# winddori2002/DEX-TTS

Hardware: AMD Instinct MI355X
Metric: mel-frames/s at n_timesteps=50, 80-ch mel (sampler only); RTF (higher is better)
Workload: dtype bf16; 1 GPU; gedex_b1: gedex_lj B=1/GPU T=512 n_timesteps=50 (BASELINE.json configs[1]); global_batch=1, frames=512, hipgraph=True, parallelism=1 GPU

## Files before the change

### dex_tts_amd/csrc/dex_api.hip

```cpp
#include <hip/hip_runtime.h>
#include <cstdlib>

#include <cmath>
#include <cstdarg>
#include <atomic>
#include <cstdio>
#include <mutex>
#include <cstring>
#include <map>
#include <unordered_map>
#include <string_view>
#include <string>
#include <vector>

#include "../../include/dex_amd.h"
#include "kernels.h"
#include "weight_store.h"

using namespace dex;

namespace dex {
namespace {
const char* const KNOB_NAMES[] = {
    "DEX_CONV_STREAM", "DEX_CONV_PP", "DEX_CONV_SKIP_DEAD", "DEX_H_BF16", "DEX_ATTN_SEPARATE", "DEX_ATTN_Q64", "DEX_ATTN_Q64_TAIL", "DEX_ATTN_Q64_HALF", "DEX_DIT_XCDS", "DEX_ATTN_GENERIC", "DEX_RES2", "DEX_LP_INTER", "DEX_DIT_CHAIN",
    "DEX_DIT_CLUSTER", "DEX_DIT_CLUSTER_LOCAL", "DEX_ATTN_X_LP", "DEX_RES_X_LP", "DEX_CAT_LP", "DEX_XCD_MAP", "DEX_DEBUG_DROP_HANDOFF", "DEX_PATCH_FUSED",
    "DEX_CONV_DOWN", "DEX_CONVT_UP", "DEX_DEBUG_PLAN",
    "DEX_ATTN_SHARED_W8", "DEX_CONVT_MT", "DEX_CONVT_WGS", "DEX_CONV_DOWN_WGS", "DEX_CONV_REGW", "DEX_CONV_REGW_RES", "DEX_CONV_SMALL_MAX", "DEX_CONV_TH8",
    "DEX_CONV_W8", "DEX_DWCONV_CAP", "DEX_FINAL_CAP", "DEX_FIRST_CAP", "DEX_FIRST_MFMA", "DEX_GEMM_NWALK", "DEX_NWALK_SPLIT", "DEX_NWALK_BM", "DEX_POS_COL", "DEX_POS_COL_MIN",
    "DEX_POS_CT", "DEX_REGW_MIN_TILES", "DEX_REGW_WGS", "DEX_ROWCHAIN64", "DEX_ROWCHAIN64A", "DEX_TIV_CAP", "DEX_TV_CHAIN", "DEX_TIV_FOLD", "DEX_LINATTN_NSUB", "DEX_TV_FOLD", "DEX_OUT2_MIN", "DEX_NWALK_DMA"};
constexpr int N_KNOBS = (int)(sizeof(KNOB_NAMES) / sizeof(KNOB_NAMES[0]));
int knob_parse(const char* e) {
    if (!e) return KNOB_UNSET;
    char* end = nullptr;
    const long v = strtol(e, &end, 10);
    if (end == e) {
        static bool warned = false;
        if (!warned) { warned = true; fprintf(stderr, "libdexamd: ignoring a DEX_* knob whose value '%s' is not an integer\n", e); }
        return KNOB_UNSET;
    }
    return (int)v;
}
struct KnobSnapshot {
    int v[N_KNOBS];
    KnobSnapshot() { for (int i = 0; i < N_KNOBS; ++i) v[i] = knob_parse(getenv(KNOB_NAMES[i])); }
};
thread_local const KnobSnapshot* t_knobs = nullptr;
struct WsplitScope {
    bool prev;
    explicit WsplitScope(bool on) : prev(g_lp_wsplit) { g_lp_wsplit = on; }
    ~WsplitScope() { g_lp_wsplit = prev; }
};
struct KnobScope {
    const KnobSnapshot* prev;
    explicit KnobScope(const KnobSnapshot* k) : prev(t_knobs) { t_knobs = k; }
    ~KnobScope() { t_knobs = prev; }
};
}
static int knob_index(const char* name) {
    static const std::unordered_map<std::string_view, int> idx = [] {
        std::unordered_map<std::string_view, int> m;
        for (int i = 0; i < N_KNOBS; ++i) m.emplace(KNOB_NAMES[i], i);
        return m;
    }();
    const auto it = idx.find(std::string_view(name));
    return it == idx.end() ? -1 : it->second;
}
int knob(const char* name) {
    if (t_knobs) {
        const int i = knob_index(name);
        if (i >= 0) return t_knobs->v[i];
    }
    return knob_parse(getenv(name));
}
}
static_assert(PREC_FP32 == DEX_PREC_FP32 && PREC_BF16 == DEX_PREC_BF16 && PREC_FP16 == DEX_PREC_FP16 && PREC_FP16X2 == DEX_PREC_FP16X2, "kernels.h mirrors DexPrecision");

namespace {
void xcd_map_probe();

struct TD { float* p; int ld; int coff; int C; int lp = 0; };

struct ResW { const float *w1, *b1, *g1, *be1, *w2, *b2, *g2, *be2, *wr, *br, *mlp_w, *mlp_b; int cin, cout; };
// ... 856 lines not shown
        if (tail) {
            tail->H2 = s.h2; tail->gn_stats = st2; tail->gamma = w.g2; tail->beta = w.be2;
            tail->res = resptr; tail->ldres = ldres; tail->resb = resb; tail->res_under_mask = under ? 1 : 0;
            tail->res_lp = (head && head->xout_lp && resptr == X.p) ? 1 : 0;
            tail->mask = mask; tail->mask_ws = s.mask_ws; tail->mask_bstride = P.d.T; tail->W = s.W; tail->Xout = out;
            tail->h2_bf16 = h2b ? 1 : 0;
            return;
        }
        gn_apply(s.h2, w.cout, npix, s.W, s.mask_ws, st2, w.g2, w.be2, nullptr, resptr, ldres, resb, under, out);
    }

    bool lp_inter_cur = false;
    bool cat_lp = false;
    IGemmP final_gemm(int mask_ws, float* out, int ldo, int ocoff) {
        const DexConfig& c = x->cfg;
        const int hid = c.dit_hidden, mid = mid_dim(c);
        const bool fuse_lnf = x->lp() && ln_fusable(hid);
        const int s2c = c.dit_stride * c.dit_stride * mid;
        IGemmP fl = base_gemm(fuse_lnf ? P.tok : P.xn, hid, 0, P.Hf, P.Wt, hid, x->fl_w, s2c, x->fl_b, out, ldo, ocoff);
        if (fuse_lnf) { fl.ln_shift = P.fin_mod; fl.ln_scale = P.fin_mod + hid; fl.ln_step_stride = 2L * hid; }
        { auto it = x->frag_of().find(x->fl_w); fl.Wfrag = (it != x->frag_of().end()) ? it->second : nullptr; }
        fl.unpatch_s = c.dit_stride; fl.unpatch_C = mid; fl.OHf = P.Hm; fl.OWf = P.Wm;
        fl.c_bstride = (long)P.Hm * P.Wm * ldo;
        fl.outmask = mask; fl.outmask_ws = mask_ws;
        return fl;
    }
    bool linattn_fused(int C) const { return x->lp() && (C == 64 || C == 128) && linattn_fused_supported(C); }
    void linattn(const LinW& w, const StageBuf& s, const TD& X, float* out, int ldo, int ocoff, const LinKvCtxP* tail = nullptr, bool out_lp = false,
                 void* out2_lp = nullptr, int ldo2 = 0, int ocoff2 = 0) {
        const long npix = s.npix; const int B = P.d.B;
        if (linattn_fused(X.C)) {
            int nsub = 1;
            while (nsub < 4 && (npix + 128 * nsub - 1) / (128 * nsub) * B > 192) nsub *= 2;
            {
                const int ncu = device_cus();
                const long slots = (long)(X.C == 64 ? 2 : 1) * ncu;
                if ((npix + 127) / 128 * B >= 2 * slots) {
                    long best = -1;
                    for (int n = 1; n <= 8; ++n) {
                        const long wgs = (npix + 128L * n - 1) / (128L * n) * B;
                        const long cost = (wgs + slots - 1) / slots * n;
                        if (best < 0 || cost <= best) { best = cost; nsub = n; }
                    }
                }
                const int forced = knob_or("DEX_LINATTN_NSUB", 0);
                if (forced > 0) nsub = forced;
            }
            const int nblk = (int)((npix + 128L * nsub - 1) / (128L * nsub));
            LinKvCtxP k{};
            if (tail) k = *tail;
            k.X = X.p; k.ldx = X.ld; k.x_coff = X.coff; k.xb = npix * X.ld; k.npix = (int)npix; k.C = X.C; k.Wkv = w.wkv_lp[x->lpi()];
            k.wkv_lo_off = x->lpi() == 2 ? 384L * X.C : 0;
            k.nsub = nsub; k.nblk = nblk; k.part_m = s.pm; k.part_s = s.ps; k.part_c = s.pc; k.B = B;
            const bool xlp = k.H2 && k.Xout && lp_inter_cur && linattn_out2_lp_out_supported((int)npix, B) && !knob_off("DEX_ATTN_X_LP");
            k.xout_lp = xlp ? 1 : 0;
            run("linattn_kvctx", 2.0 * npix * B * (256.0 * X.C + 128 * 32), (tail ? (tail->h2_bf16 ? 10.0 : 12.0) - (xlp ? 2.0 : 0.0) : 4.0) * npix * X.C * B, [&] { launch_linattn_kvctx(k, x->precision, st); });
            LinMergeP mg{s.pm, s.ps, s.pc, nblk, w.wout_raw, w.g, X.C, s.mbf, B};
            run("linattn_merge", 2.0 * 128 * 32 * X.C * B, 4.0 * nblk * 4 * 1088 * B, [&] { launch_linattn_merge(mg, x->precision, st); });
            LinOut2P o{X.p, X.ld, X.coff, npix * X.ld, (int)npix, X.C, w.wq_frag[x->lpi()], s.mbf, w.bias_eff, out, ldo, ocoff, npix * ldo, B, out_lp ? 1 : 0,
                       out2_lp, ldo2, ocoff2, npix * ldo2, xlp ? 1 : 0};
            o.wq_lo_off = x->lpi() == 2 ? 128L * X.C : 0;
            run("linattn_out", 4.0 * npix * B * 128.0 * X.C, ((out_lp ? 6.0 : 8.0) - (xlp ? 2.0 : 0.0) + (out2_lp ? 2.0 : 0.0)) * npix * X.C * B, [&] { launch_linattn_out2(o, x->precision, st); });
            return;
        }
        IGemmP g = base_gemm(X.p, X.ld, X.coff, s.H, s.W, X.C, w.wqkv, 384, nullptr, s.qkv, 384, 0);
        gemm("linattn_qkv", g);
        LinAttnCtxP cp{s.qkv, 384, npix * 384, (int)npix, 4, LA_CHUNK, s.nchunks, s.pm, s.ps, s.pc, B};
        run("linattn_ctx", 2.0 * npix * 128 * 32 * B, 4.0 * npix * 384 * B, [&] { launch_linattn_ctx(cp, st); });
        LinAttnCombineP cb{s.pm, s.ps, s.pc, s.nchunks, 4, w.wout_raw, w.g, w.C, s.weff, B};
        run("linattn_combine", 2.0 * 128 * 32 * w.C * B, 4.0 * s.nchunks * 4 * 1100 * B, [&] { launch_linattn_combine(cb, st); });
        IGemmP o = base_gemm(s.qkv, 384, 0, s.H, s.W, 128, s.weff, w.C, w.bias_eff, out, ldo, ocoff);
        o.w_bstride = 128L * w.C;
        o.res = X.p; o.ldres = X.ld; o.res_coff = X.coff; o.res_bstride = npix * X.ld;
        gemm("linattn_out", o);
    }

    void dit(const TD& X, bool mask_input, int mask_ws, float* out, int ldo, int ocoff, const float* in_aff = nullptr) {
        const DexConfig& c = x->cfg;
        const int B = P.d.B, hid = c.dit_hidden, mid = mid_dim(c), N = P.N, mh = mlp_hidden(c);
        DwConvP dw{};
        dw.X = X.p + X.coff; dw.ldx = X.ld; dw.xb = (long)P.Hm * P.Wm * X.ld; dw.Hi = P.Hm; dw.Wi = P.Wm; dw.C = mid;
        dw.k = c.dit_patch; dw.s = c.dit_stride; dw.pad = c.dit_patch / 2; dw.Wd = x->pe_dw; dw.bd = x->pe_db;
        dw.mask = mask_input ? mask : nullptr; dw.mask_ws = mask_ws; dw.mask_bstride = P.d.T;
        dw.Y = P.pe0; dw.Hf = P.Hf; dw.Wt = P.Wt; dw.B = B; dw.aff = in_aff;
        auto pw_lp = x->lp_of().find(x->pe_pw);
        if (patch_fused()) {
            run("patch_embed", 2.0 * B * N * mid * (c.dit_patch * c.dit_patch + hid), 4.0 * B * (P.Hm * P.Wm * mid + N * hid),
                [&] { launch_patch_embed_fused(dw, pw_lp->second, x->pe_pb, P.emb, hid, x->precision, st); });
        } else {
            run("patch_dwconv_silu", 2.0 * B * N * mid * c.dit_patch * c.dit_patch, 4.0 * B * (P.Hm * P.Wm + N) * mid, [&] { launch_dwconv_silu(dw, st); });
            IGemmP pe = base_gemm(P.pe0, mid, 0, P.Hf, P.Wt, mid, x->pe_pw, hid, x->pe_pb, P.emb, hid, 0);
            gemm("patch_pointwise", pe);
        }
        const int G = c.dit_conv_pos_groups, kp = c.dit_conv_pos, cg = hid / G;
        int nsplit = POS_SPLIT, pcg = 0, pcgp = 0;
        if (x->lp() && x->pos_wfrag[x->lpi()]) {
            PosConvP pcd{P.emb, x->pos_wfrag[x->lpi()], P.pos_part, P.Hf, P.Wt, hid, G, B};
            run("pos_conv", 2.0 * B * N * (double)kp * kp * cg * hid, 8.0 * B * N * hid + 2.0 * kp * kp * cg * hid, [&] { launch_pos_conv_direct(pcd, x->precision, st); });
            nsplit = 1;
        } else {
            const int cgp = (cg % 32) ? 64 : cg;
            const float* src = P.emb;
            if (cgp != cg) {
                run("pos_group_pad", 0, 8.0 * B * N * hid, [&] { launch_group_pad(P.emb, P.emb_pad, (long)B * N, G, cg, cgp, st); });
                src = P.emb_pad;
            }
// ... 821 lines not shown
```

### dex_tts_amd/csrc/kernels.h

```cpp
#pragma once
#include <hip/hip_runtime.h>
#include <stdint.h>

namespace dex {

constexpr int KNOB_UNSET = -2147483647 - 1;
int knob(const char* name);
inline int knob_or(const char* name, int dflt) { const int v = knob(name); return v == KNOB_UNSET ? dflt : v; }
inline bool knob_off(const char* name) { return knob(name) == 0; }
inline bool knob_set(const char* name) { return knob(name) != KNOB_UNSET; }
inline int device_cus() {
    static const int n = [] { int dev = 0, v = 0; (void)hipGetDevice(&dev); (void)hipDeviceGetAttribute(&v, hipDeviceAttributeMultiprocessorCount, dev); return v > 0 ? v : 256; }();
    return n;
}

constexpr int GN_SLOTS = 32;
typedef long long gnfix_t;

extern thread_local const char* g_last_symbol;

constexpr int PREC_FP32 = 0, PREC_BF16 = 1, PREC_FP16 = 2, PREC_FP16X2 = 3;
inline bool prec_wsplit(int precision) { return precision == PREC_FP16X2; }
extern thread_local bool g_lp_wsplit;
inline bool prec_is_lp(int precision) { return precision != PREC_FP32; }
// ... 86 lines not shown

struct GnStatsP { const float* X; int ld; long bstride; int npix; int C; int groups; gnfix_t* stats; int B; };
void launch_gn_stats(const GnStatsP& p, hipStream_t st);

struct GnApplyP {
    const float* X; int ldx; long xb;
    float* Y; int ldy; long yb; int y_coff;
    int npix, W, C, groups; const gnfix_t* stats; const float* gamma; const float* beta;
    const float* mask; int mask_ws; long mask_bstride;
    const float* tadd; long tadd_step_stride; int step;
    const float* res; int ldres; long resb; int res_under_mask;
    int B;
};
void launch_gn_apply(const GnApplyP& p, hipStream_t st);

struct FinalP {
    const float* X; long xb; int npix, W, C, groups; const gnfix_t* stats; const float* gamma; const float* beta;
    const float* mask; long mask_bstride;
    const float* wfc; const float* bfc;
    const float* xcur;
    float* denoised;
    float* xnext;
    const float* scal; int scal_stride; int step;
    float* zero_ptr; long zero_n;
    int B;
    int mode; const float* htab; float* dbuf; const float* xhat;
    int x_bf16;
    const int* poison;
};
void launch_final(const FinalP& p, hipStream_t st);
void launch_churn_tables(const float* sigmas, int n, float S_churn, float S_min, float S_max, float S_noise,
                         float* t_hat, float* h, float* ncoef, hipStream_t st);
void launch_add_noise(float* x, const float* noise, const float* ncoef_i, long n, hipStream_t st);
void launch_heun_expand(const float* t_hat, const float* h, int n, float* sig, float* hout, hipStream_t st);

struct LinAttnCtxP { const float* qkv; int ld; long bstride; int n; int heads; int chunk; int nchunks;
                     float* part_m; float* part_s; float* part_c; int B; };
void launch_linattn_ctx(const LinAttnCtxP& p, hipStream_t st);
struct LinAttnCombineP { const float* part_m; const float* part_s; const float* part_c; int nchunks; int heads;
                         const float* Wout;
                         const float* g;
                         int C; float* Weff;
                         int B; };
void launch_linattn_combine(const LinAttnCombineP& p, hipStream_t st);

struct LinKvCtxP { const float* X; int ldx; int x_coff; long xb; int npix; int C; const void* Wkv; int nsub; int nblk;
                   float* part_m; float* part_s; float* part_c; int B;
                   const float* H2; const gnfix_t* gn_stats; const float* gamma; const float* beta;
                   const float* res; int ldres; long resb; int res_under_mask;
                   const float* mask; int mask_ws; long mask_bstride; int W; float* Xout;
                   int h2_bf16;
                   int res_lp;
                   int xout_lp;     long wkv_lo_off = 0;
};
void launch_linattn_kvctx(const LinKvCtxP& p, int precision, hipStream_t st);
struct LinMergeP { const float* part_m; const float* part_s; const float* part_c; int nblk;
                   const float* Wout; const float* g; int C; void* W2; int B; };
void launch_linattn_merge(const LinMergeP& p, int precision, hipStream_t st);
struct LinOut2P { const float* X; int ldx; int x_coff; long xb; int npix; int C; const void* Wq; const void* W2;
                  const float* bias; float* Y; int ldy; int y_coff; long yb; int B;
                  int y_lp;
                  void* Y2; int ldy2; int y2_coff; long y2b;
                  int x_lp;     long wq_lo_off = 0;
                  };
void launch_linattn_out2(const LinOut2P& p, int precision, hipStream_t st);
bool linattn_out2_lp_out_supported(int npix, int B);
bool linattn_fused_supported(int C);

struct DwConvP { const float* X; int ldx; long xb; int Hi, Wi, C; int k, s, pad; const float* Wd; const float* bd;
                 const float* mask; int mask_ws; long mask_bstride;
                 float* Y; int Hf, Wt; int B;
                 const float* aff = nullptr; };
void launch_dwconv_silu(const DwConvP& p, hipStream_t st);
bool patch_embed_fused_supported(int k, int C, int hid, long ntok);
void launch_patch_embed_fused(const DwConvP& p, const void* Wb, const float* bias, float* emb, int hid, int precision, hipStream_t st);

struct PosConvP { const float* X; const void* Wf; float* Y; int Hf, Wt, hid, G, B;
                  int ncol; };
bool pos_conv_direct_supported(int hid, int groups, int kernel, int Hf);
void launch_pos_conv_direct(const PosConvP& p, int precision, hipStream_t st);
struct PosFinishP { const float* part; int nsplit; long split_stride; const float* bias; const float* emb;
                    const float* freq_pos; float* tok; int Hf, Wt, D; int B;
                    int cg, cg_pad; };
void launch_pos_finish(const PosFinishP& p, hipStream_t st);
void launch_group_pad(const float* src, float* dst, long rows, int G, int cg, int cg_pad, hipStream_t st);

struct LnModP { const float* X; float* Y; int rows_per_batch; int D; const float* shift; const float* scale;
                long step_stride; int step; int B; };
void launch_ln_mod(const LnModP& p, hipStream_t st);

struct DitChainP { const float* O; int ksplit; long o_sstride; const float* ml; int heads; int rows_per_batch;
                   float* X; const void *Wp, *W1, *W2, *Wq; const float *bp, *b1, *b2, *bq;
                   const float* ada;
                   const float *next_shift, *next_scale; long next_step_stride;
                   void *Qh, *Kh, *Vt; int Npad; float qscale;
                   const void *Qin, *Kin, *Vin;
                   int qkv_only;
                   int attn_inline;
                   int step; int M; int B; long long* dbg;
                   float* xslab; unsigned* xflag; unsigned epoch; int* xerr;
                   int o_lp;
                   int xcd_map;
                   int xlocal;
                   int xdrop;
                   int tail_row0 = 0, tail_ks = 0;
                   int xcds = 8; };
// ... 154 lines not shown
```

### dex_tts_amd/csrc/linattn_fused.hip

```cpp
#include "kernels.h"
#include "lp_util.h"
#include "kernels_lp.h"

namespace dex {
namespace DEX_LP_NS {

typedef float f32x16 __attribute__((ext_vector_type(16)));
typedef unsigned short u16;
union LFrag { uint4 u; lp8 v; };
constexpr float LOG2E_F = 1.4426950408889634f;


template <int C, bool PRO, int FL = -1>
__global__ __launch_bounds__(256) __attribute__((amdgpu_waves_per_eu(C == 64 ? 2 : 1, C == 64 ? 2 : 8))) void linattn_kvctx_kernel(const LinKvCtxP p) {
    constexpr int LDW = C + 8, KS = C / 16;
    extern __shared__ __attribute__((aligned(16))) u16 smem_la[];
    u16* Ws = smem_la;
    const int tid = threadIdx.x, lane = tid & 63, wave = tid >> 6;
    const int i = lane & 31, hh = lane >> 5;
    const int blk = blockIdx.x, b = blockIdx.y;
    const u16* Wg = reinterpret_cast<const u16*>(p.Wkv);
    {
        uint4 wr[C / 8];
#pragma unroll
        for (int j = 0; j < C / 8; ++j) {
            const int it = tid + 256 * j;
            wr[j] = *reinterpret_cast<const uint4*>(Wg + (long)(it / (C / 8)) * C + (it % (C / 8)) * 8);
        }
#pragma unroll
        for (int j = 0; j < C / 8; ++j) {
            const int it = tid + 256 * j;
            *reinterpret_cast<uint4*>(Ws + (it / (C / 8)) * LDW + (it % (C / 8)) * 8) = wr[j];
        }
#ifdef DEX_LP_WSPLIT
#pragma unroll
        for (int j = 0; j < C / 8; ++j) {
            const int it = tid + 256 * j;
            wr[j] = *reinterpret_cast<const uint4*>(Wg + p.wkv_lo_off + (long)(it / (C / 8)) * C + (it % (C / 8)) * 8);
        }
#pragma unroll
        for (int j = 0; j < C / 8; ++j) {
            const int it = tid + 256 * j;
            *reinterpret_cast<uint4*>(Ws + 256 * LDW + (it / (C / 8)) * LDW + (it % (C / 8)) * 8) = wr[j];
        }
#endif
    }
    const float* X = PRO ? p.H2 + (long)b * p.npix * C : p.X + (long)b * p.xb + p.x_coff;
    const int ldx = PRO ? C : p.ldx;
    const float* R = (PRO && p.res) ? p.res + (long)b * p.resb : nullptr;
    const float* mrow = PRO ? p.mask + (long)b * p.mask_bstride : nullptr;
    const int px_base = (blk * 4 + wave) * p.nsub * 32;

    f32x16 ctxT[4];
    float m_run[4], s_run[4];
#pragma unroll
    for (int h = 0; h < 4; ++h) {
        m_run[h] = -INFINITY; s_run[h] = 0.f;
#pragma unroll
        for (int r = 0; r < 16; ++r) ctxT[h][r] = 0.f;
    }
    float4 xa[KS], xc[KS], ra[PRO ? KS : 1], rc[PRO ? KS : 1];
    float mkv = 1.f;
    float ga_pre = 0.f, be_pre = 0.f;
    if constexpr (PRO) { if (tid < C) { ga_pre = p.gamma[tid]; be_pre = p.beta[tid]; } }
    const bool hb = FL >= 0 ? (FL & 1) != 0 : (PRO && p.h2_bf16 != 0);
    const bool rlp = FL >= 0 ? (FL & 2) != 0 : (PRO && p.res_lp != 0);
    const bool xlp = FL >= 0 ? (FL & 4) != 0 : (p.xout_lp != 0);
    const unsigned short* Rh = (PRO && p.res) ? reinterpret_cast<const unsigned short*>(p.res) + (long)b * p.resb : nullptr;
    const unsigned short* Xh = PRO ? reinterpret_cast<const unsigned short*>(p.H2) + (long)b * p.npix * C : nullptr;
    {
        const int pxr = min(px_base + i, p.npix - 1);
        const float* xr = X + (long)pxr * ldx + hh * 8;
        if (hb) {
#pragma unroll
            for (int ks = 0; ks < KS; ++ks) { xa[ks] = *reinterpret_cast<const float4*>(Xh + (long)pxr * C + hh * 8 + ks * 16); xc[ks] = xa[ks]; }
        } else {
#pragma unroll
            for (int ks = 0; ks < KS; ++ks) {
                xa[ks] = *reinterpret_cast<const float4*>(xr + ks * 16);
                xc[ks] = *reinterpret_cast<const float4*>(xr + ks * 16 + 4);
            }
        }
        if constexpr (PRO) {
            if (R) {
                if (rlp) {
#pragma unroll
                    for (int ks = 0; ks < KS; ++ks) { ra[ks] = *reinterpret_cast<const float4*>(Rh + (long)pxr * p.ldres + hh * 8 + ks * 16); rc[ks] = ra[ks]; }
                } else {
                    const float* rr = R + (long)pxr * p.ldres + hh * 8;
#pragma unroll
                    for (int ks = 0; ks < KS; ++ks) {
                        ra[ks] = *reinterpret_cast<const float4*>(rr + ks * 16);
                        rc[ks] = *reinterpret_cast<const float4*>(rr + ks * 16 + 4);
                    }
                }
            }
            mkv = mrow[(pxr % p.W) * p.mask_ws];
        }
    }
    __shared__ float smean[8], srstd[8];
    __shared__ __attribute__((aligned(16))) float gsc_s[PRO ? C : 4], gsh_s[PRO ? C : 4];
    if constexpr (PRO) {
        {
            const int g = tid / GN_SLOTS;
            const longlong2 sv = *reinterpret_cast<const longlong2*>(p.gn_stats + (((long)b * 8 + g) * GN_SLOTS + (tid % GN_SLOTS)) * 2);
            long long s1 = sv.x, s2 = sv.y;
            gn_slots_reduce<GN_SLOTS>(s1, s2);
            if ((tid % GN_SLOTS) == 0) gn_moments(s1, s2, 1e-5, smean[g], srstd[g]);
        }
    }
    __syncthreads();
    if constexpr (PRO) {
        if (tid < C) {
            const float ga = ga_pre * srstd[tid / (C / 8)];
            gsc_s[tid] = ga;
            gsh_s[tid] = be_pre - smean[tid / (C / 8)] * ga;
        }
        __syncthreads();
    }
    for (int sub = 0; sub < p.nsub; ++sub) {
        const int px0 = px_base + sub * 32;
        if (px0 >= p.npix) break;
        if constexpr (PRO) {
            const bool under = FL >= 0 ? (FL & 8) != 0 : (p.res_under_mask != 0);
            const bool live = px0 + i < p.npix;
            float* xo = p.Xout + ((long)b * p.npix + min(px0 + i, p.npix - 1)) * C + hh * 8;
#pragma unroll
            for (int ks = 0; ks < KS; ++ks) {
                float v[8] = {xa[ks].x, xa[ks].y, xa[ks].z, xa[ks].w, xc[ks].x, xc[ks].y, xc[ks].z, xc[ks].w};
                if (hb) {
                    const unsigned u0 = __float_as_uint(xa[ks].x), u1 = __float_as_uint(xa[ks].y), u2 = __float_as_uint(xa[ks].z), u3 = __float_as_uint(xa[ks].w);
                    v[0] = lp_lo(u0); v[1] = lp_hi(u0); v[2] = lp_lo(u1); v[3] = lp_hi(u1);
                    v[4] = lp_lo(u2); v[5] = lp_hi(u2); v[6] = lp_lo(u3); v[7] = lp_hi(u3);
                }
                float r_[8] = {0.f, 0.f, 0.f, 0.f, 0.f, 0.f, 0.f, 0.f};
                const float4 sc0 = *reinterpret_cast<const float4*>(gsc_s + ks * 16 + hh * 8), sc1 = *reinterpret_cast<const float4*>(gsc_s + ks * 16 + hh * 8 + 4);
                const float4 sh0 = *reinterpret_cast<const float4*>(gsh_s + ks * 16 + hh * 8), sh1 = *reinterpret_cast<const float4*>(gsh_s + ks * 16 + hh * 8 + 4);
                const float gsc[8] = {sc0.x, sc0.y, sc0.z, sc0.w, sc1.x, sc1.y, sc1.z, sc1.w};
                const float gsh[8] = {sh0.x, sh0.y, sh0.z, sh0.w, sh1.x, sh1.y, sh1.z, sh1.w};
                if (R) {
                    if (rlp) {
                        const unsigned u0 = __float_as_uint(ra[ks].x), u1 = __float_as_uint(ra[ks].y), u2 = __float_as_uint(ra[ks].z), u3 = __float_as_uint(ra[ks].w);
                        r_[0] = lp_lo(u0); r_[1] = lp_hi(u0); r_[2] = lp_lo(u1); r_[3] = lp_hi(u1); r_[4] = lp_lo(u2); r_[5] = lp_hi(u2); r_[6] = lp_lo(u3); r_[7] = lp_hi(u3);
                    } else { r_[0] = ra[ks].x; r_[1] = ra[ks].y; r_[2] = ra[ks].z; r_[3] = ra[ks].w; r_[4] = rc[ks].x; r_[5] = rc[ks].y; r_[6] = rc[ks].z; r_[7] = rc[ks].w; }
                }
#pragma unroll
                for (int j = 0; j < 8; ++j) {
                    const float t = fmaf(v[j], gsc[j], gsh[j]);
                    const float e = __expf(fminf(t, 20.f));
                    const float n = e * (e + 2.f);
                    const float y = t * (n * __builtin_amdgcn_rcpf(n + 2.f));
                    v[j] = under ? (y + r_[j]) * mkv : fmaf(y, mkv, r_[j]);
                }
                xa[ks] = make_float4(v[0], v[1], v[2], v[3]); xc[ks] = make_float4(v[4], v[5], v[6], v[7]);
                if (live) {
                    if (xlp) {
                        u16* xh = reinterpret_cast<u16*>(p.Xout) + ((long)b * p.npix + min(px0 + i, p.npix - 1)) * C + hh * 8 + ks * 16;
                        *reinterpret_cast<uint4*>(xh) = make_uint4(pack2_lp(v[0], v[1]), pack2_lp(v[2], v[3]), pack2_lp(v[4], v[5]), pack2_lp(v[6], v[7]));
                    } else {
                        *reinterpret_cast<float4*>(xo + ks * 16) = xa[ks];
                        *reinterpret_cast<float4*>(xo + ks * 16 + 4) = xc[ks];
                    }
                }
            }
        }
        LFrag af[KS];
#pragma unroll
        for (int ks = 0; ks < KS; ++ks) {
            af[ks].u.x = pack2_lp(xa[ks].x, xa[ks].y); af[ks].u.y = pack2_lp(xa[ks].z, xa[ks].w);
            af[ks].u.z = pack2_lp(xc[ks].x, xc[ks].y); af[ks].u.w = pack2_lp(xc[ks].z, xc[ks].w);
        }
        if (sub + 1 < p.nsub) {
            const int pxr = min(px0 + 32 + i, p.npix - 1);
            const float* xr = X + (long)pxr * ldx + hh * 8;
            if (hb) {
#pragma unroll
                for (int ks = 0; ks < KS; ++ks) { xa[ks] = *reinterpret_cast<const float4*>(Xh + (long)pxr * C + hh * 8 + ks * 16); xc[ks] = xa[ks]; }
            } else {
#pragma unroll
                for (int ks = 0; ks < KS; ++ks) {
                    xa[ks] = *reinterpret_cast<const float4*>(xr + ks * 16);
                    xc[ks] = *reinterpret_cast<const float4*>(xr + ks * 16 + 4);
                }
            }
            if constexpr (PRO) {
                if (R) {
                    if (rlp) {
#pragma unroll
                        for (int ks = 0; ks < KS; ++ks) { ra[ks] = *reinterpret_cast<const float4*>(Rh + (long)pxr * p.ldres + hh * 8 + ks * 16); rc[ks] = ra[ks]; }
                    } else {
                        const float* rr = R + (long)pxr * p.ldres + hh * 8;
#pragma unroll
                        for (int ks = 0; ks < KS; ++ks) {
                            ra[ks] = *reinterpret_cast<const float4*>(rr + ks * 16);
                            rc[ks] = *reinterpret_cast<const float4*>(rr + ks * 16 + 4);
                        }
                    }
                }
                mkv = mrow[(pxr % p.W) * p.mask_ws];
            }
        }
        constexpr bool SEED = C == 128 || (FL >= 0 && (FL & 2) != 0);
        f32x16 kseed;
#pragma unroll
        for (int r = 0; r < 16; ++r) kseed[r] = (SEED && px0 + (r & 3) + 8 * (r >> 2) + 4 * hh >= p.npix) ? -INFINITY : 0.f;
#pragma unroll
        for (int h = 0; h < 4; ++h) {
            f32x16 kh, vh;
#pragma unroll
            for (int r = 0; r < 16; ++r) { kh[r] = SEED ? kseed[r] : 0.f; vh[r] = 0.f; }
            const u16* bk = Ws + (h * 32 + i) * LDW + hh * 8;
            const u16* bv = Ws + ((4 + h) * 32 + i) * LDW + hh * 8;
#pragma unroll
            for (int ks = 0; ks < KS; ++ks) {
                LFrag fk, fv; fk.u = *reinterpret_cast<const uint4*>(bk + ks * 16); fv.u = *reinterpret_cast<const uint4*>(bv + ks * 16);
                kh = DEX_MFMA_LP(af[ks].v, fk.v, kh, 0, 0, 0);
                vh = DEX_MFMA_LP(af[ks].v, fv.v, vh, 0, 0, 0);
#ifdef DEX_LP_WSPLIT
                LFrag lk, lv; lk.u = *reinterpret_cast<const uint4*>(bk + 256 * LDW + ks * 16); lv.u = *reinterpret_cast<const uint4*>(bv + 256 * LDW + ks * 16);
                kh = DEX_MFMA_LP(af[ks].v, lk.v, kh, 0, 0, 0);
                vh = DEX_MFMA_LP(af[ks].v, lv.v, vh, 0, 0, 0);
#endif
            }
            float mx = -INFINITY;
#pragma unroll
            for (int r = 0; r < 16; ++r) {
                if constexpr (!SEED) { if (px0 + (r & 3) + 8 * (r >> 2) + 4 * hh >= p.npix) kh[r] = -INFINITY; }
                mx = fmaxf(mx, kh[r]);
            }
            mx = fmaxf(mx, __shfl_xor(mx, 32));
            constexpr float KSHIFT = LP_IS_F16 ? 14.f * 0.69314718056f : 0.f;
            const float mn = fmaxf(m_run[h], mx - KSHIFT);
            const float alpha = __expf(m_run[h] - mn);
            m_run[h] = mn;
            const float nmn2 = -mn * LOG2E_F;
            float ps = 0.f;
#pragma unroll
            for (int r = 0; r < 16; ++r) { kh[r] = __builtin_amdgcn_exp2f(fmaf(kh[r], LOG2E_F, nmn2)); ps += kh[r]; }
            s_run[h] = s_run[h] * alpha + ps;
#pragma unroll
            for (int r = 0; r < 16; ++r) ctxT[h][r] *= alpha;
#pragma unroll
            for (int k2 = 0; k2 < 2; ++k2) {
                LFrag va, pb;
                va.u.x = pack2_lp(vh[8 * k2 + 0], vh[8 * k2 + 1]); va.u.y = pack2_lp(vh[8 * k2 + 2], vh[8 * k2 + 3]);
                va.u.z = pack2_lp(vh[8 * k2 + 4], vh[8 * k2 + 5]); va.u.w = pack2_lp(vh[8 * k2 + 6], vh[8 * k2 + 7]);
                pb.u.x = pack2_lp(kh[8 * k2 + 0], kh[8 * k2 + 1]); pb.u.y = pack2_lp(kh[8 * k2 + 2], kh[8 * k2 + 3]);
                pb.u.z = pack2_lp(kh[8 * k2 + 4], kh[8 * k2 + 5]); pb.u.w = pack2_lp(kh[8 * k2 + 6], kh[8 * k2 + 7]);
                ctxT[h] = DEX_MFMA_LP(va.v, pb.v, ctxT[h], 0, 0, 0);
            }
            __builtin_amdgcn_sched_barrier(0);
        }
    }
    __syncthreads();
    float* mS = reinterpret_cast<float*>(smem_la);
    float* mm = mS + 4 * 4 * 32 * 33;
    float* ms = mm + 4 * 4 * 32;
#pragma unroll
    for (int h = 0; h < 4; ++h) {
        const float st = s_run[h] + __shfl_xor(s_run[h], 32);
        float* dst = mS + ((wave * 4 + h) * 32 + i) * 33;
#pragma unroll
        for (int r = 0; r < 16; ++r) dst[(r & 3) + 8 * (r >> 2) + 4 * hh] = ctxT[h][r];
        if (hh == 0) { mm[(wave * 4 + h) * 32 + i] = m_run[h]; ms[(wave * 4 + h) * 32 + i] = st; }
    }
    __syncthreads();
    for (int idx = tid; idx < 4 * 1024; idx += 256) {
        const int h = idx >> 10, d = (idx >> 5) & 31, e = idx & 31;
        float M = -INFINITY;
#pragma unroll
        for (int w = 0; w < 4; ++w) M = fmaxf(M, mm[(w * 4 + h) * 32 + d]);
        float acc = 0.f, s = 0.f;
#pragma unroll
        for (int w = 0; w < 4; ++w) {
            const float mw = mm[(w * 4 + h) * 32 + d];
            const float f = (mw == -INFINITY) ? 0.f : __expf(mw - M);
            acc = fmaf(f, mS[((w * 4 + h) * 32 + d) * 33 + e], acc);
            s = fmaf(f, ms[(w * 4 + h) * 32 + d], s);
        }
        const long pidx = ((long)b * 4 + h) * p.nblk + blk;
        p.part_c[pidx * 1024 + d * 32 + e] = acc;
        if (e == 0) { p.part_m[pidx * 32 + d] = M; p.part_s[pidx * 32 + d] = s; }
    }
}

void launch_linattn_kvctx(const LinKvCtxP& p, hipStream_t st) {
#ifdef DEX_LP_WSPLIT
    const size_t lds_w = (size_t)2 * 256 * (p.C + 8) * sizeof(u16);
    constexpr int LDS_MAX = 144 * 1024;
#else
    const size_t lds_w = (size_t)256 * (p.C + 8) * sizeof(u16);
    constexpr int LDS_MAX = 96 * 1024;
#endif
    const size_t lds_m = (size_t)(4 * 4 * 32 * 33 + 2 * 4 * 4 * 32) * sizeof(float);
    const size_t lds = lds_w > lds_m ? lds_w : lds_m;
    static bool attr = false;
    if (!attr) {
        hipFuncSetAttribute(reinterpret_cast<const void*>(&linattn_kvctx_kernel<64, false>), hipFuncAttributeMaxDynamicSharedMemorySize, LDS_MAX);
        hipFuncSetAttribute(reinterpret_cast<const void*>(&linattn_kvctx_kernel<128, false>), hipFuncAttributeMaxDynamicSharedMemorySize, LDS_MAX);
        hipFuncSetAttribute(reinterpret_cast<const void*>(&linattn_kvctx_kernel<64, true>), hipFuncAttributeMaxDynamicSharedMemorySize, LDS_MAX);
        hipFuncSetAttribute(reinterpret_cast<const void*>(&linattn_kvctx_kernel<128, true>), hipFuncAttributeMaxDynamicSharedMemorySize, LDS_MAX);
#define KVCTX_ATTR(CC, F) hipFuncSetAttribute(reinterpret_cast<const void*>(&linattn_kvctx_kernel<CC, true, F>), hipFuncAttributeMaxDynamicSharedMemorySize, LDS_MAX);
        KVCTX_ATTR(64, 1) KVCTX_ATTR(64, 3) KVCTX_ATTR(64, 5) KVCTX_ATTR(64, 7) KVCTX_ATTR(64, 9) KVCTX_ATTR(64, 11) KVCTX_ATTR(64, 13) KVCTX_ATTR(64, 15)
        KVCTX_ATTR(128, 1) KVCTX_ATTR(128, 3) KVCTX_ATTR(128, 5) KVCTX_ATTR(128, 7) KVCTX_ATTR(128, 9) KVCTX_ATTR(128, 11) KVCTX_ATTR(128, 13) KVCTX_ATTR(128, 15)
#undef KVCTX_ATTR
        attr = true;
    }
    dim3 grid(p.nblk, p.B);
    const bool pro = p.H2 != nullptr;
    const int fl = pro ? (p.h2_bf16 != 0 ? 1 : 0) | (p.res_lp != 0 ? 2 : 0) | (p.xout_lp != 0 ? 4 : 0) | (p.res_under_mask != 0 ? 8 : 0) : -1;
#define KVCTX_CASE(CC, F) case F: hipLaunchKernelGGL((linattn_kvctx_kernel<CC, true, F>), grid, dim3(256), lds, st, p); break;
#define KVCTX_LAUNCH(CC)                                                                                                              \
    switch (fl) {                                                                                                                      \
        KVCTX_CASE(CC, 1) KVCTX_CASE(CC, 3) KVCTX_CASE(CC, 5) KVCTX_CASE(CC, 7) KVCTX_CASE(CC, 9) KVCTX_CASE(CC, 11) KVCTX_CASE(CC, 13) KVCTX_CASE(CC, 15)   \
        default:                                                                                                                       \
            if (pro) hipLaunchKernelGGL((linattn_kvctx_kernel<CC, true>), grid, dim3(256), lds, st, p);                                \
            else hipLaunchKernelGGL((linattn_kvctx_kernel<CC, false>), grid, dim3(256), lds, st, p);                                   \
    }
    if (p.C == 64) { KVCTX_LAUNCH(64) } else { KVCTX_LAUNCH(128) }
#undef KVCTX_LAUNCH
#undef KVCTX_CASE
}

template <int MC>
__device__ __forceinline__ void merge_fold(const LinMergeP& p, long pbase, int d, int e, int pl, float& m, float& acc, float& s) {
    for (int c0 = 0; c0 < p.nblk; c0 += 8 * MC) {
        float pm[MC], ps[MC], pc[MC];
#pragma unroll
        for (int k = 0; k < MC; ++k) {
            const int c = min(c0 + pl + 8 * k, p.nblk - 1);
            pm[k] = p.part_m[(pbase + c) * 32 + d];
            ps[k] = p.part_s[(pbase + c) * 32 + d];
            pc[k] = p.part_c[(pbase + c) * 1024 + d * 32 + e];
        }
#pragma unroll
        for (int k = 0; k < MC; ++k) {
            if (c0 + pl + 8 * k < p.nblk) {
                const float mn = fmaxf(m, pm[k]);
                const float a = (m == -INFINITY) ? 0.f : __expf(m - mn);
                const float w = (pm[k] == -INFINITY) ? 0.f : __expf(pm[k] - mn);
                acc = fmaf(acc, a, w * pc[k]);
                s = fmaf(s, a, w * ps[k]);
                m = mn;
            }
        }
    }
}

__global__ __launch_bounds__(256) void linattn_merge_kernel(const LinMergeP p) {
    __shared__ float redm[8], reda[8][32], reds[8], cvec[32];
    const int tid = threadIdx.x, h = blockIdx.x, b = blockIdx.y, d = blockIdx.z;
    const int C = p.C;
    float4 wo[8];
    if (tid < C) {
#pragma unroll
        for (int j = 0; j < 8; ++j) wo[j] = *reinterpret_cast<const float4*>(p.Wout + (long)tid * 128 + h * 32 + j * 4);
    }
    const float g = p.g[0];
    const long pbase = ((long)b * 4 + h) * p.nblk;
    const int e = tid & 31, pl = tid >> 5;
    float m = -INFINITY, acc = 0.f, s = 0.f;
    const int per_lane = (p.nblk + 7) / 8;
    if (per_lane <= 8) merge_fold<8>(p, pbase, d, e, pl, m, acc, s);
    else if (per_lane <= 16) merge_fold<16>(p, pbase, d, e, pl, m, acc, s);
    else merge_fold<24>(p, pbase, d, e, pl, m, acc, s);
    if (e == 0) { redm[pl] = m; reds[pl] = s; }
    reda[pl][e] = acc;
    __syncthreads();
    if (pl == 0) {
        float M = redm[0];
#pragma unroll
// ... 258 lines not shown
```

Baseline: 25900 mel-frames/s.

## Add head-parallel 1024-thread linear-attention KV-context kernel for small grids

```diff
diff --git a/dex_tts_amd/csrc/dex_api.hip b/dex_tts_amd/csrc/dex_api.hip
--- a/dex_tts_amd/csrc/dex_api.hip
+++ b/dex_tts_amd/csrc/dex_api.hip
@@ -27,7 +27,8 @@
     "DEX_CONV_DOWN", "DEX_CONVT_UP", "DEX_DEBUG_PLAN",
     "DEX_ATTN_SHARED_W8", "DEX_CONVT_MT", "DEX_CONVT_WGS", "DEX_CONV_DOWN_WGS", "DEX_CONV_REGW", "DEX_CONV_REGW_RES", "DEX_CONV_SMALL_MAX", "DEX_CONV_TH8",
     "DEX_CONV_W8", "DEX_DWCONV_CAP", "DEX_FINAL_CAP", "DEX_FIRST_CAP", "DEX_FIRST_MFMA", "DEX_GEMM_NWALK", "DEX_NWALK_SPLIT", "DEX_NWALK_BM", "DEX_POS_COL", "DEX_POS_COL_MIN",
-    "DEX_POS_CT", "DEX_REGW_MIN_TILES", "DEX_REGW_WGS", "DEX_ROWCHAIN64", "DEX_ROWCHAIN64A", "DEX_TIV_CAP", "DEX_TV_CHAIN", "DEX_TIV_FOLD", "DEX_LINATTN_NSUB", "DEX_TV_FOLD", "DEX_OUT2_MIN", "DEX_NWALK_DMA"};
+    "DEX_POS_CT", "DEX_REGW_MIN_TILES", "DEX_REGW_WGS", "DEX_ROWCHAIN64", "DEX_ROWCHAIN64A", "DEX_TIV_CAP", "DEX_TV_CHAIN", "DEX_TIV_FOLD", "DEX_LINATTN_NSUB", "DEX_TV_FOLD", "DEX_OUT2_MIN", "DEX_NWALK_DMA",
+    "DEX_LINATTN_HEADWAVES"};
 constexpr int N_KNOBS = (int)(sizeof(KNOB_NAMES) / sizeof(KNOB_NAMES[0]));
 int knob_parse(const char* e) {
     if (!e) return KNOB_UNSET;
@@ -990,6 +991,7 @@
             k.X = X.p; k.ldx = X.ld; k.x_coff = X.coff; k.xb = npix * X.ld; k.npix = (int)npix; k.C = X.C; k.Wkv = w.wkv_lp[x->lpi()];
             k.wkv_lo_off = x->lpi() == 2 ? 384L * X.C : 0;
             k.nsub = nsub; k.nblk = nblk; k.part_m = s.pm; k.part_s = s.ps; k.part_c = s.pc; k.B = B;
+            k.headwaves = knob_or("DEX_LINATTN_HEADWAVES", (long)nblk * B <= device_cus() ? 1 : 0) != 0 ? 1 : 0;
             const bool xlp = k.H2 && k.Xout && lp_inter_cur && linattn_out2_lp_out_supported((int)npix, B) && !knob_off("DEX_ATTN_X_LP");
             k.xout_lp = xlp ? 1 : 0;
             run("linattn_kvctx", 2.0 * npix * B * (256.0 * X.C + 128 * 32), (tail ? (tail->h2_bf16 ? 10.0 : 12.0) - (xlp ? 2.0 : 0.0) : 4.0) * npix * X.C * B, [&] { launch_linattn_kvctx(k, x->precision, st); });
diff --git a/dex_tts_amd/csrc/kernels.h b/dex_tts_amd/csrc/kernels.h
--- a/dex_tts_amd/csrc/kernels.h
+++ b/dex_tts_amd/csrc/kernels.h
@@ -162,6 +162,8 @@
                    int h2_bf16;
                    int res_lp;
                    int xout_lp;     long wkv_lo_off = 0;
+                   int headwaves = 0;
+                   long long* dbg = nullptr;
 };
 void launch_linattn_kvctx(const LinKvCtxP& p, int precision, hipStream_t st);
 struct LinMergeP { const float* part_m; const float* part_s; const float* part_c; int nblk;
diff --git a/dex_tts_amd/csrc/linattn_fused.hip b/dex_tts_amd/csrc/linattn_fused.hip
--- a/dex_tts_amd/csrc/linattn_fused.hip
+++ b/dex_tts_amd/csrc/linattn_fused.hip
@@ -10,12 +10,120 @@
 union LFrag { uint4 u; lp8 v; };
 constexpr float LOG2E_F = 1.4426950408889634f;
 
+
+#ifdef DEX_TIMING
+#define KSTAMP_DECL long long tk[8] = {0, 0, 0, 0, 0, 0, 0, 0}; const long long tk0 = __builtin_readcyclecounter(); long long tlast = tk0;
+#define KSTAMP(k) do { const long long now_ = __builtin_readcyclecounter(); tk[k] += now_ - tlast; tlast = now_; } while (0)
+#define KSTAMP_STORE(n)                                                                                               \
+    if (p.dbg && threadIdx.x == 0) {                                                                                  \
+        long long* d_ = p.dbg + ((long)blockIdx.y * gridDim.x + blockIdx.x) * 8;                                      \
+        for (int k_ = 0; k_ < (n); ++k_) d_[k_] = tk[k_];                                                             \
+        d_[7] = __builtin_readcyclecounter() - tk0;                                                                   \
+    }
+#else
+#define KSTAMP_DECL
+#define KSTAMP(k) do {} while (0)
+#define KSTAMP_STORE(n)
+#endif
+
+__device__ __forceinline__ void kv_prologue8(const LinKvCtxP& p, float4& xa, float4& xc, const float4& ra, const float4& rc, const float* gsc_s,
+                                             const float* gsh_s, int ch, bool hb, bool rlp, bool has_r, bool under, bool xlp, float mkv,
+                                             bool live, long orow) {
+#pragma clang fp contract(on)
+    float v[8] = {xa.x, xa.y, xa.z, xa.w, xc.x, xc.y, xc.z, xc.w};
+    if (hb) {
+        const unsigned u0 = __float_as_uint(xa.x), u1 = __float_as_uint(xa.y), u2 = __float_as_uint(xa.z), u3 = __float_as_uint(xa.w);
+        v[0] = lp_lo(u0); v[1] = lp_hi(u0); v[2] = lp_lo(u1); v[3] = lp_hi(u1);
+        v[4] = lp_lo(u2); v[5] = lp_hi(u2); v[6] = lp_lo(u3); v[7] = lp_hi(u3);
+    }
+    float r_[8] = {0.f, 0.f, 0.f, 0.f, 0.f, 0.f, 0.f, 0.f};
+    const float4 sc0 = *reinterpret_cast<const float4*>(gsc_s + ch), sc1 = *reinterpret_cast<const float4*>(gsc_s + ch + 4);
+    const float4 sh0 = *reinterpret_cast<const float4*>(gsh_s + ch), sh1 = *reinterpret_cast<const float4*>(gsh_s + ch + 4);
+    const float gsc[8] = {sc0.x, sc0.y, sc0.z, sc0.w, sc1.x, sc1.y, sc1.z, sc1.w};
+    const float gsh[8] = {sh0.x, sh0.y, sh0.z, sh0.w, sh1.x, sh1.y, sh1.z, sh1.w};
+    if (has_r) {
+        if (rlp) {
+            const unsigned u0 = __float_as_uint(ra.x), u1 = __float_as_uint(ra.y), u2 = __float_as_uint(ra.z), u3 = __float_as_uint(ra.w);
+            r_[0] = lp_lo(u0); r_[1] = lp_hi(u0); r_[2] = lp_lo(u1); r_[3] = lp_hi(u1); r_[4] = lp_lo(u2); r_[5] = lp_hi(u2); r_[6] = lp_lo(u3); r_[7] = lp_hi(u3);
+        } else { r_[0] = ra.x; r_[1] = ra.y; r_[2] = ra.z; r_[3] = ra.w; r_[4] = rc.x; r_[5] = rc.y; r_[6] = rc.z; r_[7] = rc.w; }
+    }
+#pragma unroll
+    for (int j = 0; j < 8; ++j) {
+        const float t = fmaf(v[j], gsc[j], gsh[j]);
+        const float e = __expf(fminf(t, 20.f));
+        const float n = e * (e + 2.f);
+        const float q = n * __builtin_amdgcn_rcpf(n + 2.f);
+        v[j] = under ? fmaf(t, q, r_[j]) * mkv : fmaf(t * q, mkv, r_[j]);
+    }
+    xa = make_float4(v[0], v[1], v[2], v[3]); xc = make_float4(v[4], v[5], v[6], v[7]);
+    if (live) {
+        if (xlp) {
+            u16* xh = reinterpret_cast<u16*>(p.Xout) + orow * p.C + ch;
+            *reinterpret_cast<uint4*>(xh) = make_uint4(pack2_lp(v[0], v[1]), pack2_lp(v[2], v[3]), pack2_lp(v[4], v[5]), pack2_lp(v[6], v[7]));
+        } else {
+            float* xo = p.Xout + orow * p.C + ch;
+            *reinterpret_cast<float4*>(xo) = xa;
+            *reinterpret_cast<float4*>(xo + 4) = xc;
+        }
+    }
+}
+
+template <int C, bool SEED, int KG = 0>
+__device__ __forceinline__ void kv_head_step(const u16* Ws, int h, int i, int hh, const LFrag* af, const f32x16& kseed, int px0, int npix,
+                                             f32x16& ctx, float& m_run, float& s_run) {
+    constexpr int LDW = C + 8, KS = C / 16;
+    f32x16 kh, vh;
+#pragma unroll
+    for (int r = 0; r < 16; ++r) { kh[r] = SEED ? kseed[r] : 0.f; vh[r] = 0.f; }
+    const u16* bk = Ws + (h * 32 + i) * LDW + hh * 8;
+    const u16* bv = Ws + ((4 + h) * 32 + i) * LDW + hh * 8;
+#pragma unroll
+    for (int ks = 0; ks < KS; ++ks) {
+        LFrag fk, fv; fk.u = *reinterpret_cast<const uint4*>(bk + ks * 16); fv.u = *reinterpret_cast<const uint4*>(bv + ks * 16);
+        kh = DEX_MFMA_LP(af[ks].v, fk.v, kh, 0, 0, 0);
+        vh = DEX_MFMA_LP(af[ks].v, fv.v, vh, 0, 0, 0);
+#ifdef DEX_LP_WSPLIT
+        LFrag lk, lv; lk.u = *reinterpret_cast<const uint4*>(bk + 256 * LDW + ks * 16); lv.u = *reinterpret_cast<const uint4*>(bv + 256 * LDW + ks * 16);
+        kh = DEX_MFMA_LP(af[ks].v, lk.v, kh, 0, 0, 0);
+        vh = DEX_MFMA_LP(af[ks].v, lv.v, vh, 0, 0, 0);
+#endif
+        if constexpr (KG > 0) { if ((ks + 1) % KG == 0) __builtin_amdgcn_sched_barrier(0); }
+    }
+    float mx = -INFINITY;
+#pragma unroll
+    for (int r = 0; r < 16; ++r) {
+        if constexpr (!SEED) { if (px0 + (r & 3) + 8 * (r >> 2) + 4 * hh >= npix) kh[r] = -INFINITY; }
+        mx = fmaxf(mx, kh[r]);
+    }
+    mx = fmaxf(mx, __shfl_xor(mx, 32));
+    constexpr float KSHIFT = LP_IS_F16 ? 14.f * 0.69314718056f : 0.f;
+    const float mn = fmaxf(m_run, mx - KSHIFT);
+    const float alpha = __expf(m_run - mn);
+    m_run = mn;
+    const float nmn2 = -mn * LOG2E_F;
+    float ps = 0.f;
+#pragma unroll
+    for (int r = 0; r < 16; ++r) { kh[r] = __builtin_amdgcn_exp2f(fmaf(kh[r], LOG2E_F, nmn2)); ps += kh[r]; }
+    s_run = s_run * alpha + ps;
+#pragma unroll
+    for (int r = 0; r < 16; ++r) ctx[r] *= alpha;
+#pragma unroll
+    for (int k2 = 0; k2 < 2; ++k2) {
+        LFrag va, pb;
+        va.u.x = pack2_lp(vh[8 * k2 + 0], vh[8 * k2 + 1]); va.u.y = pack2_lp(vh[8 * k2 + 2], vh[8 * k2 + 3]);
+        va.u.z = pack2_lp(vh[8 * k2 + 4], vh[8 * k2 + 5]); va.u.w = pack2_lp(vh[8 * k2 + 6], vh[8 * k2 + 7]);
+        pb.u.x = pack2_lp(kh[8 * k2 + 0], kh[8 * k2 + 1]); pb.u.y = pack2_lp(kh[8 * k2 + 2], kh[8 * k2 + 3]);
+        pb.u.z = pack2_lp(kh[8 * k2 + 4], kh[8 * k2 + 5]); pb.u.w = pack2_lp(kh[8 * k2 + 6], kh[8 * k2 + 7]);
+        ctx = DEX_MFMA_LP(va.v, pb.v, ctx, 0, 0, 0);
+    }
+}
 
 template <int C, bool PRO, int FL = -1>
 __global__ __launch_bounds__(256) __attribute__((amdgpu_waves_per_eu(C == 64 ? 2 : 1, C == 64 ? 2 : 8))) void linattn_kvctx_kernel(const LinKvCtxP p) {
     constexpr int LDW = C + 8, KS = C / 16;
     extern __shared__ __attribute__((aligned(16))) u16 smem_la[];
     u16* Ws = smem_la;
+    KSTAMP_DECL
     const int tid = threadIdx.x, lane = tid & 63, wave = tid >> 6;
     const int i = lane & 31, hh = lane >> 5;
     const int blk = blockIdx.x, b = blockIdx.y;
@@ -98,6 +206,7 @@
             mkv = mrow[(pxr % p.W) * p.mask_ws];
         }
     }
+    KSTAMP(0);
     __shared__ float smean[8], srstd[8];
     __shared__ __attribute__((aligned(16))) float gsc_s[PRO ? C : 4], gsh_s[PRO ? C : 4];
     if constexpr (PRO) {
@@ -118,6 +227,7 @@
         }
         __syncthreads();
     }
+    KSTAMP(1);
     for (int sub = 0; sub < p.nsub; ++sub) {
         const int px0 = px_base + sub * 32;
         if (px0 >= p.npix) break;
@@ -200,6 +310,7 @@
                 mkv = mrow[(pxr % p.W) * p.mask_ws];
             }
         }
+        KSTAMP(2);
         constexpr bool SEED = C == 128 || (FL >= 0 && (FL & 2) != 0);
         f32x16 kseed;
 #pragma unroll
@@ -251,6 +362,7 @@
             }
             __builtin_amdgcn_sched_barrier(0);
         }
+        KSTAMP(4);
     }
     __syncthreads();
     float* mS = reinterpret_cast<float*>(smem_la);
@@ -265,6 +377,7 @@
         if (hh == 0) { mm[(wave * 4 + h) * 32 + i] = m_run[h]; ms[(wave * 4 + h) * 32 + i] = st; }
     }
     __syncthreads();
+    KSTAMP(5);
     for (int idx = tid; idx < 4 * 1024; idx += 256) {
         const int h = idx >> 10, d = (idx >> 5) & 31, e = idx & 31;
         float M = -INFINITY;
@@ -282,6 +395,219 @@
         p.part_c[pidx * 1024 + d * 32 + e] = acc;
         if (e == 0) { p.part_m[pidx * 32 + d] = M; p.part_s[pidx * 32 + d] = s; }
     }
+    KSTAMP(6);
+    KSTAMP_STORE(7)
+}
+
+template <int C, bool PRO, int FL = -1>
+__global__ __launch_bounds__(1024) void linattn_kvctx_hw_kernel(const LinKvCtxP p) {
+    constexpr int LDW = C + 8, KS = C / 16, KQ = KS / 4;
+#ifdef DEX_LP_WSPLIT
+    constexpr int NWI = 2;
+#else
+    constexpr int NWI = 1;
+#endif
+    extern __shared__ __attribute__((aligned(16))) u16 smem_la[];
+    u16* Ws = smem_la;
+    u16* Xs = smem_la + NWI * 256 * LDW;
+    KSTAMP_DECL
+    const int tid = threadIdx.x, lane = tid & 63, wave = tid >> 6;
+    const int hd = wave & 3, slot = wave >> 2;
+    const int i = lane & 31, hh = lane >> 5;
+    const int blk = blockIdx.x, b = blockIdx.y;
+    const u16* Wg = reinterpret_cast<const u16*>(p.Wkv);
+    {
+        uint4 wr[C / 32];
+#pragma unroll
+        for (int j = 0; j < C / 32; ++j) {
+            const int it = tid + 1024 * j;
+            wr[j] = *reinterpret_cast<const uint4*>(Wg + (long)(it / (C / 8)) * C + (it % (C / 8)) * 8);
+        }
+#pragma unroll
+        for (int j = 0; j < C / 32; ++j) {
+            const int it = tid + 1024 * j;
+            *reinterpret_cast<uint4*>(Ws + (it / (C / 8)) * LDW + (it % (C / 8)) * 8) = wr[j];
+        }
+#ifdef DEX_LP_WSPLIT
+#pragma unroll
+        for (int j = 0; j < C / 32; ++j) {
+            const int it = tid + 1024 * j;
+            wr[j] = *reinterpret_cast<const uint4*>(Wg + p.wkv_lo_off + (long)(it / (C / 8)) * C + (it % (C / 8)) * 8);
+        }
+#pragma unroll
+        for (int j = 0; j < C / 32; ++j) {
+            const int it = tid + 1024 * j;
+            *reinterpret_cast<uint4*>(Ws + 256 * LDW + (it / (C / 8)) * LDW + (it % (C / 8)) * 8) = wr[j];
+        }
+#endif
+    }
+    const float* X = PRO ? p.H2 + (long)b * p.npix * C : p.X + (long)b * p.xb + p.x_coff;
+    const int ldx = PRO ? C : p.ldx;
+    const float* R = (PRO && p.res) ? p.res + (long)b * p.resb : nullptr;
+    const float* mrow = PRO ? p.mask + (long)b * p.mask_bstride : nullptr;
+    const int px_base = (blk * 4 + slot) * p.nsub * 32;
+    const int ch0 = hd * KQ * 16 + hh * 8;
+
+    f32x16 ctxT;
+    float m_run = -INFINITY, s_run = 0.f;
+#pragma unroll
+    for (int r = 0; r < 16; ++r) ctxT[r] = 0.f;
+    float4 xa[KQ], xc[KQ], ra[PRO ? KQ : 1], rc[PRO ? KQ : 1];
+    float mkv = 1.f;
+    float ga_pre = 0.f, be_pre = 0.f;
+    if constexpr (PRO) { if (tid < C) { ga_pre = p.gamma[tid]; be_pre = p.beta[tid]; } }
+    const bool hb = FL >= 0 ? (FL & 1) != 0 : (PRO && p.h2_bf16 != 0);
+    const bool rlp = FL >= 0 ? (FL & 2) != 0 : (PRO && p.res_lp != 0);
+    const bool xlp = FL >= 0 ? (FL & 4) != 0 : (p.xout_lp != 0);
+    const unsigned short* Rh = (PRO && p.res) ? reinterpret_cast<const unsigned short*>(p.res) + (long)b * p.resb : nullptr;
+    const unsigned short* Xh = PRO ? reinterpret_cast<const unsigned short*>(p.H2) + (long)b * p.npix * C : nullptr;
+    auto load_rows = [&](int px0) {
+        const int pxr = min(px0 + i, p.npix - 1);
+        if (hb) {
+#pragma unroll
+            for (int ks = 0; ks < KQ; ++ks) { xa[ks] = *reinterpret_cast<const float4*>(Xh + (long)pxr * C + ch0 + ks * 16); xc[ks] = xa[ks]; }
+        } else {
+            const float* xr = X + (long)pxr * ldx + ch0;
+#pragma unroll
+            for (int ks = 0; ks < KQ; ++ks) {
+                xa[ks] = *reinterpret_cast<const float4*>(xr + ks * 16);
+                xc[ks] = *reinterpret_cast<const float4*>(xr + ks * 16 + 4);
+            }
+        }
+        if constexpr (PRO) {
+            if (R) {
+                if (rlp) {
+#pragma unroll
+                    for (int ks = 0; ks < KQ; ++ks) { ra[ks] = *reinterpret_cast<const float4*>(Rh + (long)pxr * p.ldres + ch0 + ks * 16); rc[ks] = ra[ks]; }
+                } else {
+                    const float* rr = R + (long)pxr * p.ldres + ch0;
+#pragma unroll
+                    for (int ks = 0; ks < KQ; ++ks) {
+                        ra[ks] = *reinterpret_cast<const float4*>(rr + ks * 16);
+                        rc[ks] = *reinterpret_cast<const float4*>(rr + ks * 16 + 4);
+                    }
+                }
+            }
+            mkv = mrow[(pxr % p.W) * p.mask_ws];
+        }
+    };
+    load_rows(px_base);
+    KSTAMP(0);
+    __shared__ float smean[8], srstd[8];
+    __shared__ __attribute__((aligned(16))) float gsc_s[PRO ? C : 4], gsh_s[PRO ? C : 4];
+    if constexpr (PRO) {
+        if (tid < 256) {
+            const int g = tid / GN_SLOTS;
+            const longlong2 sv = *reinterpret_cast<const longlong2*>(p.gn_stats + (((long)b * 8 + g) * GN_SLOTS + (tid % GN_SLOTS)) * 2);
+            long long s1 = sv.x, s2 = sv.y;
+            gn_slots_reduce<GN_SLOTS>(s1, s2);
+            if ((tid % GN_SLOTS) == 0) gn_moments(s1, s2, 1e-5, smean[g], srstd[g]);
+        }
+    }
+    __syncthreads();
+    if constexpr (PRO) {
+        if (tid < C) {
+            const float ga = ga_pre * srstd[tid / (C / 8)];
+            gsc_s[tid] = ga;
+            gsh_s[tid] = be_pre - smean[tid / (C / 8)] * ga;
+        }
+        __syncthreads();
+    }
+    KSTAMP(1);
+    constexpr bool SEED = C == 128 || (FL >= 0 && (FL & 2) != 0);
+    for (int sub = 0; sub < p.nsub; ++sub) {
+        const int px0 = px_base + sub * 32;
+        const bool act = px0 < p.npix;
+        u16* xs = Xs + ((slot * 2 + (sub & 1)) * 32 + i) * LDW;
+        if (act) {
+            if constexpr (PRO) {
+                const bool under = FL >= 0 ? (FL & 8) != 0 : (p.res_under_mask != 0);
+                const bool live = px0 + i < p.npix;
+                const long orow = (long)b * p.npix + min(px0 + i, p.npix - 1);
+#pragma unroll
+                for (int ks = 0; ks < KQ; ++ks)
+                    kv_prologue8(p, xa[ks], xc[ks], ra[ks], rc[ks], gsc_s, gsh_s, ch0 + ks * 16, hb, rlp, R != nullptr, under, xlp, mkv, live, orow);
+            }
+#pragma unroll
+            for (int ks = 0; ks < KQ; ++ks)
+                *reinterpret_cast<uint4*>(xs + ch0 + ks * 16) =
+                    make_uint4(pack2_lp(xa[ks].x, xa[ks].y), pack2_lp(xa[ks].z, xa[ks].w), pack2_lp(xc[ks].x, xc[ks].y), pack2_lp(xc[ks].z, xc[ks].w));
+            if (sub + 1 < p.nsub) load_rows(px0 + 32);
+        }
+        KSTAMP(2);
+        __syncthreads();
+        KSTAMP(3);
+        if (!act) continue;
+        LFrag af[KS];
+#pragma unroll
+        for (int ks = 0; ks < KS; ++ks) af[ks].u = *reinterpret_cast<const uint4*>(xs + ks * 16 + hh * 8);
+        f32x16 kseed;
+#pragma unroll
+        for (int r = 0; r < 16; ++r) kseed[r] = (SEED && px0 + (r & 3) + 8 * (r >> 2) + 4 * hh >= p.npix) ? -INFINITY : 0.f;
+        kv_head_step<C, SEED, (C == 128 ? 4 : 0)>(Ws, hd, i, hh, af, kseed, px0, p.npix, ctxT, m_run, s_run);
+        KSTAMP(4);
+    }
+    __syncthreads();
+    float* mS = reinterpret_cast<float*>(smem_la);
+    float* mm = mS + 4 * 4 * 32 * 33;
+    float* ms = mm + 4 * 4 * 32;
+    {
+        const float st = s_run + __shfl_xor(s_run, 32);
+        float* dst = mS + ((slot * 4 + hd) * 32 + i) * 33;
+#pragma unroll
+        for (int r = 0; r < 16; ++r) dst[(r & 3) + 8 * (r >> 2) + 4 * hh] = ctxT[r];
+        if (hh == 0) { mm[(slot * 4 + hd) * 32 + i] = m_run; ms[(slot * 4 + hd) * 32 + i] = st; }
+    }
+    __syncthreads();
+    KSTAMP(5);
+    for (int idx = tid; idx < 4 * 1024; idx += 1024) {
+        const int h = idx >> 10, d = (idx >> 5) & 31, e = idx & 31;
+        float M = -INFINITY;
+#pragma unroll
+        for (int w = 0; w < 4; ++w) M = fmaxf(M, mm[(w * 4 + h) * 32 + d]);
+        float acc = 0.f, s = 0.f;
+#pragma unroll
+        for (int w = 0; w < 4; ++w) {
+            const float mw = mm[(w * 4 + h) * 32 + d];
+            const float f = (mw == -INFINITY) ? 0.f : __expf(mw - M);
+            acc = fmaf(f, mS[((w * 4 + h) * 32 + d) * 33 + e], acc);
+            s = fmaf(f, ms[(w * 4 + h) * 32 + d], s);
+        }
+        const long pidx = ((long)b * 4 + h) * p.nblk + blk;
+        p.part_c[pidx * 1024 + d * 32 + e] = acc;
+        if (e == 0) { p.part_m[pidx * 32 + d] = M; p.part_s[pidx * 32 + d] = s; }
+    }
+    KSTAMP(6);
+    KSTAMP_STORE(7)
+}
+
+static bool kvctx_hw_supported(int C) {
+#ifdef DEX_LP_WSPLIT
+    return C == 64;
+#else
+    return C == 64 || C == 128;
+#endif
+}
+template <int CC>
+static void launch_kvctx_hw(const LinKvCtxP& p, int fl, bool pro, dim3 grid, size_t lds, hipStream_t st) {
+    constexpr int LDS_HW = 144 * 1024;
+    static bool attr = false;
+    if (!attr) {
+        hipFuncSetAttribute(reinterpret_cast<const void*>(&linattn_kvctx_hw_kernel<CC, false>), hipFuncAttributeMaxDynamicSharedMemorySize, LDS_HW);
+        hipFuncSetAttribute(reinterpret_cast<const void*>(&linattn_kvctx_hw_kernel<CC, true>), hipFuncAttributeMaxDynamicSharedMemorySize, LDS_HW);
+#define KVHW_ATTR(F) hipFuncSetAttribute(reinterpret_cast<const void*>(&linattn_kvctx_hw_kernel<CC, true, F>), hipFuncAttributeMaxDynamicSharedMemorySize, LDS_HW);
+        KVHW_ATTR(1) KVHW_ATTR(3) KVHW_ATTR(5) KVHW_ATTR(7) KVHW_ATTR(9) KVHW_ATTR(11) KVHW_ATTR(13) KVHW_ATTR(15)
+#undef KVHW_ATTR
+        attr = true;
+    }
+#define KVHW_CASE(F) case F: hipLaunchKernelGGL((linattn_kvctx_hw_kernel<CC, true, F>), grid, dim3(1024), lds, st, p); break;
+    switch (fl) {
+        KVHW_CASE(1) KVHW_CASE(3) KVHW_CASE(5) KVHW_CASE(7) KVHW_CASE(9) KVHW_CASE(11) KVHW_CASE(13) KVHW_CASE(15)
+        default:
+            if (pro) hipLaunchKernelGGL((linattn_kvctx_hw_kernel<CC, true>), grid, dim3(1024), lds, st, p);
+            else hipLaunchKernelGGL((linattn_kvctx_hw_kernel<CC, false>), grid, dim3(1024), lds, st, p);
+    }
+#undef KVHW_CASE
 }
 
 void launch_linattn_kvctx(const LinKvCtxP& p, hipStream_t st) {
@@ -309,6 +635,18 @@
     dim3 grid(p.nblk, p.B);
     const bool pro = p.H2 != nullptr;
     const int fl = pro ? (p.h2_bf16 != 0 ? 1 : 0) | (p.res_lp != 0 ? 2 : 0) | (p.xout_lp != 0 ? 4 : 0) | (p.res_under_mask != 0 ? 8 : 0) : -1;
+    if (p.headwaves && kvctx_hw_supported(p.C)) {
+        g_last_symbol = "linattn_kvctx_hw_kernel";
+        const size_t lds_hw = lds_w + (size_t)4 * 2 * 32 * (p.C + 8) * sizeof(u16);
+        const size_t lds2 = lds_hw > lds_m ? lds_hw : lds_m;
+#ifdef DEX_LP_WSPLIT
+        launch_kvctx_hw<64>(p, fl, pro, grid, lds2, st);
+#else
+        if (p.C == 64) launch_kvctx_hw<64>(p, fl, pro, grid, lds2, st);
+        else launch_kvctx_hw<128>(p, fl, pro, grid, lds2, st);
+#endif
+        return;
+    }
 #define KVCTX_CASE(CC, F) case F: hipLaunchKernelGGL((linattn_kvctx_kernel<CC, true, F>), grid, dim3(256), lds, st, p); break;
 #define KVCTX_LAUNCH(CC)                                                                                                              \
     switch (fl) {                                                                                                                      \
@@ -317,6 +655,7 @@
             if (pro) hipLaunchKernelGGL((linattn_kvctx_kernel<CC, true>), grid, dim3(256), lds, st, p);                                \
             else hipLaunchKernelGGL((linattn_kvctx_kernel<CC, false>), grid, dim3(256), lds, st, p);                                   \
     }
+    g_last_symbol = "linattn_kvctx_kernel";
     if (p.C == 64) { KVCTX_LAUNCH(64) } else { KVCTX_LAUNCH(128) }
 #undef KVCTX_LAUNCH
 #undef KVCTX_CASE
```

Result: faster. 26960 mel-frames/s, median of 6 (+4.1%).
